# daisy9542/yolo-puncture

Hardware: AMD Instinct MI355X
Metric: images/sec (higher is better)
Workload: dtype bf16

## Files before the change

### include/yolop.h

```cpp
#ifndef YOLOP_H
#define YOLOP_H

#include <stddef.h>
#include <stdint.h>

#ifdef __cplusplus
extern "C" {
#endif

#define YP_OK 0
#define YP_ERR_ARG -1
#define YP_ERR_STATE -2
#define YP_ERR_HIP -3
#define YP_ERR_WEIGHT -4

#define YP_BF16 0
#define YP_F32 1

#define YP_TASK_DETECT 0
#define YP_TASK_SEGMENT 1

#define YP_NM 32
#define YP_MAX_MASKS 480
#define YP_MAX_DET 512
// ... 120 lines not shown
int yp_profile(yp_engine* e, const uint8_t* in_dev, int B, int H, int W, float* det_out, int32_t* idx_out,
               float* coeff_out, float* ms_out, int iters, void* stream);

int yp_set_nms(yp_engine* e, float conf, float iou);

int yp_set_attention_form(yp_engine* e, int form);

int yp_set_autotune(yp_engine* e, int enable);

int yp_tuning_export(const yp_engine* e, int32_t* cfg_out, int cap);
int yp_tuning_import(yp_engine* e, int B, int H, int W, const int32_t* cfg, int n);

int yp_debug_force_conv_cfg(int cfg);
int yp_debug_op_cfg(const yp_engine* e, int i, int* cfg);
int yp_debug_last_store_form(void);
int yp_debug_max_workgroups(int n);
int yp_debug_conv_families(int* base, int* num_cfgs, int cap);
int yp_debug_ablation(int v);
int yp_debug_head_clocks(uint64_t* out8);
int yp_debug_attention(const void* qkv_dev, void* o_dev, int dtype, int B, int N, int nh, int kd, int hd, int q_stride, int q_coff, int o_stride,
                       int o_coff, int wgs, int* kernel_out, void* stream);
int yp_debug_attention_form(const void* qkv_dev, void* o_dev, int dtype, int B, int N, int nh, int kd, int hd, int q_stride, int q_coff, int o_stride,
                            int o_coff, int wgs, int form, int* kernel_out, void* stream);
int yp_debug_topk_anchors(const uint32_t* const mk_dev[3], int B, const int hw[3][2], int k, int32_t* sel_out_dev, uint32_t* thr_out_dev, void* stream);
int yp_debug_head_branch_clocks(uint64_t* out8);
int yp_debug_head_winners(yp_engine* e, int32_t* sel_host, float* box_host, float* coeff_host);
int yp_debug_contour_clocks(uint64_t* out12);
int yp_debug_pwsp_clocks(uint64_t* out32);

int yp_tuning_source(const yp_engine* e);

int yp_debug_host_selftest(yp_engine* e);
int yp_debug_graph_info(const yp_engine* e, int64_t* out6);
int yp_debug_head_positions(yp_engine* e, int64_t* out6);
int yp_debug_marker(void* stream);

int yp_set_graph(yp_engine* e, int enable);

#ifdef __cplusplus
}
#endif
#endif
```

### yolo-puncture_amd/csrc/common.h

```cpp
#pragma once
#include <hip/hip_runtime.h>
#include <stdint.h>
#include <atomic>
#include <cstdlib>
#include <string>
#include <vector>

namespace yp {

enum DType { DT_BF16 = 0, DT_F32 = 1 };
enum Act { ACT_NONE = 0, ACT_SILU = 1, ACT_RELU = 2 };

enum OpKind {
    OP_STEM = 0,
    OP_CONV = 1,
    OP_DWCONV = 2,
    OP_POOL5 = 3,
    OP_UPSAMPLE = 4,
    OP_ATTN = 5,
    OP_HEAD = 6,
    OP_CONVT = 7,
    OP_AMAX = 9,
    OP_POOL3 = 8,
};
// ... 251 lines not shown
int conv_dma_requested_cfg(const ConvParams& p);
int conv_launch_cfg(const ConvParams& p, int dtype);
void conv_dma_force_cfg(int cfg);
int conv_dma_forced_cfg();
void conv_set_debug_ablation(int v);
int conv_debug_ablation();
bool tile_balance_enabled(int family);

struct ConvFamily {
    int base, num_cfgs;
    bool (*valid)(const ConvParams& p, int c);
    std::string (*symbol)(const ConvParams& p, int c);
    hipError_t (*launch)(const ConvParams& p, int c, hipStream_t st);
    bool two_source;
    const char* tune_env;
    bool opt_in;
};
inline const char* res_f32_args(const ConvParams& p) { return p.out_f32 ? ",false,true" : p.res ? ",true,false" : ",false,false"; }
extern const ConvFamily conv_dma_family, conv_halo_family, conv_halo_p_family, conv_dma_p_family, conv_dma_lc_family, conv_halo_s2_family,
    conv_tile1_family, conv_wreg_family, conv_pxd_family, conv_ks_family, conv_wres_family, conv_wrs_family;
constexpr int kNumConvFamilies = 12;
extern const ConvFamily* const kConvFamilies[kNumConvFamilies];
int conv_halo_s2_pw_cfg(const ConvParams& p);
hipError_t launch_dwconv(const DwParams& p, int dtype, hipStream_t st);
std::string dwconv_kernel_name(const DwParams& p, int dtype);
hipError_t launch_stem(const StemParams& p, int dtype, hipStream_t st);
std::string stem_kernel_name(const StemParams& p, int dtype);
hipError_t launch_pool5(const PoolParams& p, int dtype, hipStream_t st);
hipError_t launch_sppf_pool3(const PoolParams& p, int dtype, hipStream_t st);
bool sppf_pool3_fits(const PoolParams& p, int dtype);
bool dwconv_mfma_valid(const DwParams& p, int dtype);
hipError_t launch_dwconv_mfma(const DwParams& p, hipStream_t st);
const char* dwconv_mfma_kernel_name(const DwParams& p);
hipError_t launch_upsample(const UpParams& p, int dtype, hipStream_t st);
enum AttnForm { ATTN_FORM_AUTO = 0, ATTN_FORM_STREAM = 1, ATTN_FORM_STREAM_WIDE = 3 };
inline bool attn_form_valid(int form) { return form == ATTN_FORM_AUTO || form == ATTN_FORM_STREAM || form == ATTN_FORM_STREAM_WIDE; }
constexpr int ATTN_RESIDENT_TOKENS = 400;
hipError_t launch_attention(const AttnParams& p, int dtype, hipStream_t st, int wgs = 0, int* kernel_out = nullptr, int form = ATTN_FORM_AUTO);
bool attention_fits(const AttnParams& p, int dtype, int* max_tokens, int form = ATTN_FORM_AUTO);
bool attention_takes_stream(const AttnParams& p, int dtype, int form);
bool attention_takes_stream_wide(const AttnParams& p, int dtype, int form);
bool attention_stream_scope(const AttnParams& p, int dtype);
void attention_stream_split(int B, int N, int nh, int wgs, int* nsplit_out, int* gpw_out);
hipError_t launch_attention_stream(const AttnParams& p, hipStream_t st, int wgs);
bool attention_stream_wide_scope(const AttnParams& p, int dtype);
hipError_t launch_attention_stream_wide(const AttnParams& p, hipStream_t st, int wgs);
// ... 118 lines not shown
```

### yolo-puncture_amd/csrc/conv_halo_s2.hip

```cpp
#include "common.h"

namespace yp {

template <int FM, int FN, int WGM, int WGN, int NSH, bool HAS_RES, bool OUT_F32, bool PW2>
__global__ __launch_bounds__(WGM * WGN * 64) void conv_halo_s2_kernel(const ConvParams p, const int tiles_h, const int tiles_w,
                                                                    const int ntiles, const int G) {
    constexpr int NW = WGM * WGN;
    constexpr int TH = WGM * FM, BN = WGN * FN * 16;
    constexpr int HR = 2 * TH + 1;
    constexpr int HP = HR * 33;
    constexpr int H_INSTR = (HP * 4 + 63) / 64;
    constexpr int LH = (H_INSTR + NW - 1) / NW;
    constexpr int HB = H_INSTR * 1024;
    constexpr int S = FM * FN;
    static_assert(NSH == 3, "wait selection below is written for a 3-slot ring");
    static_assert((NSH - 2) * LH + 2 * S < 64, "vmcnt immediate");

    extern __shared__ __attribute__((aligned(1024))) unsigned char smem[];
    unsigned char* const Hs = smem;
    unsigned char* const dump = smem + NSH * HB;
    unsigned char* const Wres = dump + 1024;

    const int tid = threadIdx.x, lane = tid & 63;
    const int wave = __builtin_amdgcn_readfirstlane(tid >> 6);
    const int wm = wave % WGM, wn = wave / WGM;
    const int fr = lane & 15, fc = lane >> 4;
    const int nchunk = p.Cin >> 5;

    const int bid = xcd_remap(blockIdx.x, gridDim.x);
    const int nt = bid % ntiles, j0 = bid / ntiles;
    const int n0 = nt * BN;
    const int B = p.M / (p.Ho * p.Wo);
    const int num_tiles = B * tiles_h * tiles_w;

    const __amdgpu_buffer_rsrc_t xrs = __builtin_amdgcn_make_buffer_rsrc((void*)p.x, 0, (int)p.x_bytes, 0x00020000);
    const __amdgpu_buffer_rsrc_t wrs = __builtin_amdgcn_make_buffer_rsrc((void*)p.w, 0, (int)p.w_bytes, 0x00020000);
    const __amdgpu_buffer_rsrc_t yrs = __builtin_amdgcn_make_buffer_rsrc((void*)p.y, 0, (int)p.y_bytes, 0x00020000);

    float bias[FN][4];
#pragma unroll
    for (int a = 0; a < FN; ++a) {
        const int co = n0 + wn * (FN * 16) + a * 16 + fc * 4;
#pragma unroll
        for (int r = 0; r < 4; ++r) bias[a][r] = (co + r < p.Cout) ? p.bias[co + r] : 0.f;
    }

    {
        const int rows = 9 * nchunk * BN;
        const int ninstr = rows >> 4;
        for (int ii = wave; ii < ninstr; ii += NW) {
            const int s = ii * 64 + lane;
            const int rg = s >> 2, pc = s & 3;
            const int c8 = pc ^ cswz64(rg);
            const int n = rg % BN, q = rg / BN;
            const int tap = q % 9, ch = q / 9;
            const unsigned voff = (unsigned)(((n0 + n) * p.Kpad + tap * p.Cin + ch * 32 + c8 * 8) * 2);
            __builtin_amdgcn_raw_ptr_buffer_load_lds(wrs, (lds_void*)(Wres + ii * 1024), 16, voff, 0, 0, 0);
        }
    }

    unsigned char* const W2s = Wres + (size_t)9 * nchunk * BN * 64;
    float bias2[FN][4];
    if (PW2) {
        static_assert(!PW2 || BN == 64, "the fused trailing 1x1 is written for a 64-wide intermediate and output");
        const __amdgpu_buffer_rsrc_t w2rs = __builtin_amdgcn_make_buffer_rsrc((void*)p.w2, 0, (int)p.w2_bytes, 0x00020000);
        for (int ii = wave; ii < BN * 8 / 64; ii += NW) {
            const int s = ii * 64 + lane;
            const int row = s >> 3, pc = s & 7;
            const int c8 = pc ^ ((row >> 1) & 7);
            const unsigned voff = (unsigned)((row * p.Kpad2 + c8 * 8) * 2);
            __builtin_amdgcn_raw_ptr_buffer_load_lds(w2rs, (lds_void*)(W2s + ii * 1024), 16, voff, 0, 0, 0);
        }
#pragma unroll
        for (int a = 0; a < FN; ++a) {
            const int co = wn * (FN * 16) + a * 16 + fc * 4;
#pragma unroll
            for (int r = 0; r < 4; ++r) bias2[a][r] = (co + r < p.C2) ? p.bias2[co + r] : 0.f;
        }
    }

    unsigned hconst[LH];
// ... 30 lines not shown
        it_slot = (it_slot + 1 == NSH) ? 0 : it_slot + 1;
        if (++it_c == nchunk) {
            it_c = 0;
            it_tile += G;
            set_tile(it_tile);
        }
    };

#pragma unroll
    for (int s = 0; s < NSH - 1; ++s) issue_next();
    wait_vmcnt<0>();
    __builtin_amdgcn_s_barrier();

    int rd_slot = 0;
    unsigned epmask = 0;
    bool first_iter = true;
    for (int tile = j0; tile < num_tiles; tile += G) {
        f32x4 acc[FN][FM];
#pragma unroll
        for (int a = 0; a < FN; ++a)
#pragma unroll
            for (int r = 0; r < FM; ++r) acc[a][r] = f32x4{bias[a][0], bias[a][1], bias[a][2], bias[a][3]};

        for (int c = 0; c < nchunk; ++c) {
            if (!first_iter) {
                const int k = __builtin_popcount(epmask & ((1u << (NSH - 1)) - 1u));
                if (k == 0) wait_vmcnt<(NSH - 2) * LH>();
                else if (k == 1) wait_vmcnt<(NSH - 2) * LH + S>();
                else wait_vmcnt<(NSH - 2) * LH + 2 * S>();
                __builtin_amdgcn_s_barrier();
            }
            first_iter = false;
            issue_next();
            epmask <<= 1;

            const unsigned char* hsl = Hs + rd_slot * HB;
#pragma unroll
            for (int kx = 0; kx < 3; ++kx) {
                bf16x8 wf[3][FN];
#pragma unroll
                for (int ky = 0; ky < 3; ++ky)
#pragma unroll
                    for (int a = 0; a < FN; ++a) {
                        const int rw = (c * 9 + ky * 3 + kx) * BN + wn * (FN * 16) + a * 16 + fr;
                        wf[ky][a] = *(const bf16x8*)(Wres + swz64((unsigned)(rw * 64 + fc * 16)));
                    }
                const int eoff = (kx == 1) ? 17 + fr : fr + (kx >> 1);
#pragma unroll
                for (int jj = 0; jj < 2 * FM + 1; ++jj) {
                    const int hp = (2 * wm * FM + jj) * 33 + eoff;
                    const bf16x8 xf = *(const bf16x8*)(hsl + swz64((unsigned)(hp * 64 + fc * 16)));
                    if (jj & 1) {
#pragma unroll
                        for (int a = 0; a < FN; ++a)
                            acc[a][jj >> 1] = __builtin_amdgcn_mfma_f32_16x16x32_bf16(wf[1][a], xf, acc[a][jj >> 1], 0, 0, 0);
                    } else {
                        if ((jj >> 1) < FM) {
#pragma unroll
                            for (int a = 0; a < FN; ++a)
                                acc[a][jj >> 1] = __builtin_amdgcn_mfma_f32_16x16x32_bf16(wf[0][a], xf, acc[a][jj >> 1], 0, 0, 0);
                        }
                        if ((jj >> 1) >= 1) {
#pragma unroll
                            for (int a = 0; a < FN; ++a)
                                acc[a][(jj >> 1) - 1] = __builtin_amdgcn_mfma_f32_16x16x32_bf16(wf[2][a], xf, acc[a][(jj >> 1) - 1], 0, 0, 0);
                        }
                    }
                }
            }
            rd_slot = (rd_slot + 1 == NSH) ? 0 : rd_slot + 1;
        }

        if (PW2) {
            unsigned char* tb = Hs + ((rd_slot == 0) ? NSH - 1 : rd_slot - 1) * HB;
            __builtin_amdgcn_s_barrier();
#pragma unroll
            for (int r = 0; r < FM; ++r) {
                const int px = (wm * FM + r) * 16 + fr;
#pragma unroll
                for (int a = 0; a < FN; ++a) {
                    const int co = wn * (FN * 16) + a * 16 + fc * 4;
                    __attribute__((aligned(8))) __bf16 o[4];
                    float sv[4] = {acc[a][r][0], acc[a][r][1], acc[a][r][2], acc[a][r][3]};
                    if (p.act == ACT_SILU) silu4_packed(sv);
#pragma unroll
                    for (int i = 0; i < 4; ++i) o[i] = (__bf16)sv[i];
                    asm volatile("ds_write_b64 %0, %1" ::"v"((unsigned)(size_t)(__attribute__((address_space(3))) unsigned char*)(tb + px * 128 + (((co >> 3) ^ ((px >> 1) & 7)) * 16) + (co & 7) * 2)),
                                 "v"(*(const unsigned long long*)o) : "memory");
                }
            }
            asm volatile("s_waitcnt lgkmcnt(0)" ::: "memory");
            __builtin_amdgcn_s_barrier();
#pragma unroll
// ... 51 lines not shown
                    const int co = n0 + wn * (FN * 16) + a * 16 + fc * 4;
                    const bool ok = pix_ok && (co < (PW2 ? p.C2 : p.Cout));
                    float v[4] = {acc[a][r][0], acc[a][r][1], acc[a][r][2], acc[a][r][3]};
                    if ((PW2 ? p.act2 : p.act) == ACT_SILU) silu4_packed(v);
                    if (HAS_RES) {
                        const uint2 rr = rres[r][a];
                        add_res_bf16x4(v, rr);
                    }
                    if (OUT_F32) {
                        const unsigned off = ok ? (m * (unsigned)p.y_stride + (unsigned)(p.y_coff + co)) * 4u : kBufferOOB;
                        store_f32x4(v, yrs, off);
                    } else {
                        const unsigned off = ok ? (m * (unsigned)p.y_stride + (unsigned)(p.y_coff + co)) * 2u : kBufferOOB;
                        store_bf16x4(v, yrs, off);
                    }
                }
            }
        }
        epmask |= 1u;
    }
    wait_vmcnt<0>();
}

struct HaloS2Cfg { int FM, FN, WGM, WGN; const char* name; };
static const HaloS2Cfg kS2[] = {
    {2, 2, 4, 2, "conv_halo_s2_kernel<2,2,4,2,3"},
    {1, 2, 4, 2, "conv_halo_s2_kernel<1,2,4,2,3"},
    {2, 2, 4, 1, "conv_halo_s2_kernel<2,2,4,1,3"},
    {1, 2, 4, 1, "conv_halo_s2_kernel<1,2,4,1,3"},
    {2, 4, 4, 2, "conv_halo_s2_kernel<2,4,4,2,3"},
};
constexpr int kNumS2 = (int)(sizeof(kS2) / sizeof(kS2[0]));
static std::string conv_halo_s2_symbol(const ConvParams& p, int c) {
    return std::string(kS2[c].name) + (p.C2 > 0 ? ",false,false,true>" : std::string(res_f32_args(p)) + ",false>");
}

static size_t halo_s2_lds(const HaloS2Cfg& k, int Cin, bool pw2 = false) {
    const int TH = k.WGM * k.FM, BN = k.WGN * k.FN * 16;
    const int HP = (2 * TH + 1) * 33, H_INSTR = (HP * 4 + 63) / 64;
    return (size_t)3 * H_INSTR * 1024 + 1024 + (size_t)9 * (Cin / 32) * BN * 64 + (pw2 ? (size_t)BN * 128 : 0);
}

static bool conv_halo_s2_cfg_valid(const ConvParams& p, int c) {
    if (c < 0 || c >= kNumS2) return false;
    if (p.ks != 3 || p.stride != 2 || p.pad != 1 || p.up != 1 || (p.Cin % 32) != 0 || (p.Kpad != 9 * p.Cin)) return false;
    if ((p.H & 1) || (p.W & 1) || p.Ho * 2 != p.H || p.Wo * 2 != p.W) return false;
    if (p.x_bytes >= (1ull << 31) || p.w_bytes >= (1ull << 31) || p.y_bytes >= (1ull << 31)) return false;
    if ((p.Cout & 3) || (p.y_stride & 3) || (p.y_coff & 3) || (p.res && ((p.res_stride & 3) || (p.res_coff & 3)))) return false;
    if (p.res && p.out_f32) return false;
    const HaloS2Cfg& k = kS2[c];
    const int BN = k.WGN * k.FN * 16, TH = k.WGM * k.FM;
    const int cpad = (p.Cout + 31) / 32 * 32;
    if (BN > cpad) return false;
    if (halo_s2_lds(k, p.Cin) > 160 * 1024) return false;
    const long covered = (long)((p.Ho + TH - 1) / TH * TH) * ((p.Wo + 15) / 16 * 16);
    if (covered * 2 > (long)p.Ho * p.Wo * 3) return false;
    return true;
}

template <int FM, int FN, int WGM, int WGN, bool HAS_RES, bool OUT_F32, bool PW2 = false>
static hipError_t launch_halo_s2_var(const ConvParams& p, const HaloS2Cfg& k, hipStream_t st) {
    constexpr int TH = WGM * FM, BN = WGN * FN * 16;
    const size_t sh = halo_s2_lds(k, p.Cin, PW2);
    const int B = p.M / (p.Ho * p.Wo);
    const int tiles_h = (p.Ho + TH - 1) / TH, tiles_w = (p.Wo + 15) / 16, ntiles = (p.Cout + BN - 1) / BN;
    const int num_tiles = B * tiles_h * tiles_w;
    const int per_cu = (int)std::max<size_t>(1, std::min<size_t>(2, (160 * 1024) / sh));
    int G = (256 * per_cu) / ntiles;
    if (G < 1) G = 1;
    if (G > num_tiles) G = num_tiles;
    auto kern = conv_halo_s2_kernel<FM, FN, WGM, WGN, 3, HAS_RES, OUT_F32, PW2>;
    static size_t granted = 0;
    if (hipError_t e = allow_dynamic_lds((const void*)kern, sh, granted)) return e;
    hipLaunchKernelGGL(kern, dim3(G * ntiles), dim3(WGM * WGN * 64), sh, st, p, tiles_h, tiles_w, ntiles, G);
    return hipGetLastError();
}

template <int FM, int FN, int WGM, int WGN>
static hipError_t launch_halo_s2_one(const ConvParams& p, const HaloS2Cfg& k, hipStream_t st) {
    if (p.out_f32) return launch_halo_s2_var<FM, FN, WGM, WGN, false, true>(p, k, st);
    if (p.res) return launch_halo_s2_var<FM, FN, WGM, WGN, true, false>(p, k, st);
    return launch_halo_s2_var<FM, FN, WGM, WGN, false, false>(p, k, st);
}

int conv_halo_s2_pw_cfg(const ConvParams& p) {
    if (p.w2 == nullptr && p.C2 == 0) return -1;
    if (p.Cout != 64 || p.C2 != 64 || p.Kpad2 != 64 || p.res || p.out_f32) return -1;
    for (int c : {0, 1}) {
        ConvParams q = p;
        q.Cout = p.C2;
        if (!conv_halo_s2_cfg_valid(q, c)) continue;
        if (halo_s2_lds(kS2[c], p.Cin, true) > 160 * 1024) continue;
        return c;
    }
    return -1;
}

static hipError_t launch_conv_halo_s2(const ConvParams& p, int c, hipStream_t st) {
    const HaloS2Cfg& k = kS2[c];
    if (p.C2 > 0) {
        if (c == 0) return launch_halo_s2_var<2, 2, 4, 2, false, false, true>(p, k, st);
        if (c == 1) return launch_halo_s2_var<1, 2, 4, 2, false, false, true>(p, k, st);
        return hipErrorInvalidValue;
    }
    switch (c) {
        case 0: return launch_halo_s2_one<2, 2, 4, 2>(p, k, st);
        case 1: return launch_halo_s2_one<1, 2, 4, 2>(p, k, st);
        case 2: return launch_halo_s2_one<2, 2, 4, 1>(p, k, st);
        case 3: return launch_halo_s2_one<1, 2, 4, 1>(p, k, st);
        default: return launch_halo_s2_one<2, 4, 4, 2>(p, k, st);
    }
}

#if !defined(__HIP_DEVICE_COMPILE__)
const ConvFamily conv_halo_s2_family = {500, kNumS2, conv_halo_s2_cfg_valid, conv_halo_s2_symbol, launch_conv_halo_s2, false, "YOLOP_NO_S2", false};
#endif

}
```

### yolo-puncture_amd/csrc/engine.hip

```cpp
#include "../../include/yolop.h"
#include "common.h"
#include <algorithm>
#include <array>
#include <chrono>

#include <cmath>
#include <cstdarg>
#include <cstdio>
#include <cstring>
#include <cstdlib>
#include <dlfcn.h>
#include <fcntl.h>
#include <fstream>
#include <map>
#include <sstream>
#include <memory>

using namespace yp;

static thread_local char g_err[512] = "";
static int fail(int code, const char* fmt, ...) {
    va_list ap;
    va_start(ap, fmt);
    vsnprintf(g_err, sizeof(g_err), fmt, ap);
// ... 2348 lines not shown
        return fail(YP_ERR_ARG, "yp_debug_attention: the output slice [%d, %lld) does not fit o_stride = %d", o_coff, (long long)o_coff + (long long)nh * hd, o_stride);
    if ((q_stride | q_coff | o_stride | o_coff) & 3)
        return fail(YP_ERR_ARG, "yp_debug_attention: strides and channel offsets must be multiples of 4 elements (q_stride %d, q_coff %d, o_stride %d, o_coff %d)",
                    q_stride, q_coff, o_stride, o_coff);
    AttnParams p{};
    p.qkv = qkv_dev; p.q_stride = q_stride; p.q_coff = q_coff; p.o = o_dev; p.o_stride = o_stride; p.o_coff = o_coff;
    p.B = B; p.N = N; p.nh = nh; p.kd = kd; p.hd = hd; p.scale = 1.0f / std::sqrt((float)kd);
    int max_tokens = 0;
    if (!attention_fits(p, dtype, &max_tokens, form))
        return fail(YP_ERR_ARG, "yp_debug_attention: no kernel for N = %d, kd = %d, hd = %d: the attention kernels hold at most %d tokens and want kd and hd in multiples of 4",
                    N, kd, hd, max_tokens);
    hipStream_t st = (hipStream_t)stream;
    hipError_t err = launch_attention(p, dtype, st, wgs, kernel_out, form);
    if (err == hipSuccess) err = hipStreamSynchronize(st);
    if (err != hipSuccess) return fail(YP_ERR_HIP, "yp_debug_attention: %s", hipGetErrorString(err));
    return YP_OK;
}

int yp_debug_attention(const void* qkv_dev, void* o_dev, int dtype, int B, int N, int nh, int kd, int hd, int q_stride, int q_coff, int o_stride,
                       int o_coff, int wgs, int* kernel_out, void* stream) {
    return yp_debug_attention_form(qkv_dev, o_dev, dtype, B, N, nh, kd, hd, q_stride, q_coff, o_stride, o_coff, wgs, ATTN_FORM_AUTO, kernel_out, stream);
}

int yp_tuning_source(const yp_engine* e) {
    if (!e) return YP_ERR_ARG;
    return e->tune_source;
}

int yp_debug_graph_info(const yp_engine* e, int64_t* out6) {
    if (!e || !out6) return fail(YP_ERR_ARG, "yp_debug_graph_info: null argument");
    out6[0] = e->n_captures; out6[1] = e->g_nodes; out6[2] = e->g_edges; out6[3] = e->g_edges_expected;
    out6[4] = (int64_t)e->lanes_used.size() + 1; out6[5] = e->gexec ? 1 : 0;
    return YP_OK;
}

int yp_debug_head_positions(yp_engine* e, int64_t* out6) {
    if (!e || !out6) return fail(YP_ERR_ARG, "yp_debug_head_positions: null argument");
    for (int i = 0; i < 6; ++i) out6[i] = 0;
    if (!e->allocated) return fail(YP_ERR_STATE, "no forward has run yet");
    const Op* h = nullptr;
    for (const Op& o : e->ops) if (o.kind == OP_HEAD) h = &o;
    if (!h || !(h->sparse_box || h->sparse_cf) || !e->sp_ws) return 0;
    HIPCHK(hipSetDevice(e->device));
    HIPCHK(hipDeviceSynchronize());
    const SparseWs ws = sparse_ws_layout(*e);
    const char* base = (const char*)e->sp_ws;
// ... 366 lines not shown
```

### yolo-puncture_amd/engine.py

```python
from __future__ import annotations

import ctypes as C
import os
from typing import Dict, List, Optional, Tuple

import numpy as np
import torch

from .weights import fold_state

_LIB: Optional[C.CDLL] = None
_HERE = os.path.dirname(os.path.abspath(__file__))
LIB_PATH = os.environ.get("YOLOP_LIB") or os.path.join(_HERE, "libyolop.so")

YP_BF16, YP_F32 = 0, 1
TASK_DETECT, TASK_SEGMENT = 0, 1
OP_KINDS = {0: "stem", 1: "conv", 2: "dwconv", 3: "pool5", 4: "upsample", 5: "attn", 6: "head", 7: "convT", 8: "pool3", 9: "amax"}
FORMS = ("plain", "dwpw", "dwpw_tail", "s2pw", "frontend", "c2f", "scdown", "pwsp", "cls_out")


class ModelDesc(C.Structure):
    _fields_ = [("variant", C.c_int), ("nc", C.c_int), ("task", C.c_int), ("dtype", C.c_int), ("max_det", C.c_int), ("family", C.c_int)]


# ... 21 lines not shown
    lib.yp_forward.argtypes = [vp, vp, C.c_int, C.c_int, C.c_int, vp, vp, vp, vp]
    lib.yp_proto.argtypes = [vp, C.POINTER(vp), ip, ip]
    lib.yp_masks.argtypes = [vp, C.c_int, vp, vp, C.c_int, C.c_int, C.c_int, C.c_int, vp, vp, vp, C.c_int, C.c_int, vp]
    lib.yp_id_mask_resized.argtypes = [vp, C.c_int, vp, vp] + [C.c_int] * 5 + [vp, vp, C.c_int, C.c_int, vp]
    lib.yp_id_mask_resized.restype = C.c_int
    lib.yp_mask_contours.argtypes = [vp, C.c_int, C.c_int, C.c_int, C.c_int, vp, vp, vp, vp]
    lib.yp_mask_contours.restype = C.c_int
    lib.yp_mask_contours_scaled.argtypes = [vp, C.c_int, C.c_int, C.c_int, C.c_int, C.c_int, vp, vp, vp, C.c_int, vp, C.c_int, C.c_int, vp]
    lib.yp_mask_contours_scaled.restype = C.c_int
    lib.yp_mask_contours_large_workspace.argtypes = [C.c_int, C.c_int, C.c_int]
    lib.yp_mask_contours_large_workspace.restype = C.c_size_t
    lib.yp_mask_contours_large.argtypes = [vp, C.c_int, C.c_int, C.c_int, C.c_int, C.c_int, vp, vp, vp, C.c_int, vp, C.c_int, C.c_int, C.c_int, vp,
                                           C.c_size_t, vp]
    lib.yp_mask_contours_large.restype = C.c_int
    lib.yp_plan.argtypes = [vp, C.c_int, C.c_int, C.c_int]
    lib.yp_max_batch.argtypes = [vp, C.c_int, C.c_int]
    lib.yp_max_batch.restype = C.c_int
    lib.yp_debug_topk_anchors.argtypes = [C.POINTER(vp), C.c_int, C.POINTER(C.c_int), C.c_int, vp, vp, vp]
    lib.yp_debug_topk_anchors.restype = C.c_int
    lib.yp_debug_attention.argtypes = [vp, vp] + [C.c_int] * 11 + [ip, vp]
    lib.yp_debug_attention.restype = C.c_int
    lib.yp_debug_attention_form.argtypes = [vp, vp] + [C.c_int] * 12 + [ip, vp]
    lib.yp_debug_attention_form.restype = C.c_int
    lib.yp_set_attention_form.argtypes = [vp, C.c_int]
    lib.yp_set_attention_form.restype = C.c_int
    lib.yp_op_info.argtypes = [vp, C.c_int, C.c_char_p, C.c_int, ip, C.POINTER(C.c_double), C.POINTER(C.c_double)]
    lib.yp_op_output.argtypes = [vp, C.c_int, ip, ip, ip]
    lib.yp_op_kernel.argtypes = [vp, C.c_int, C.c_char_p, C.c_int]
    lib.yp_op_fusion.argtypes = [vp, C.c_int, ip, ip]
    lib.yp_op_fusion.restype = C.c_int
    lib.yp_debug_op_form.argtypes = [vp, C.c_int, ip, ip, C.c_int]
    lib.yp_debug_op_form.restype = C.c_int
    lib.yp_run_op.argtypes = [vp, C.c_int, vp, vp, vp, vp, vp]
    lib.yp_tensor_write.argtypes = [vp, C.c_int, C.c_int, C.c_int, vp]
    lib.yp_tensor_count.argtypes = [vp]
    lib.yp_tensor_info.argtypes = [vp, C.c_int, C.c_char_p, C.c_int, ip, ip]
    lib.yp_tensor_read.argtypes = [vp, C.c_int, vp]
    lib.yp_profile.argtypes = [vp, vp, C.c_int, C.c_int, C.c_int, vp, vp, vp, vp, C.c_int, vp]
    lib.yp_set_graph.argtypes = [vp, C.c_int]
    lib.yp_set_autotune.argtypes = [vp, C.c_int]
    lib.yp_set_nms.argtypes = [vp, C.c_float, C.c_float]
    lib.yp_set_nms.restype = C.c_int
    lib.yp_debug_host_selftest.argtypes = [vp]
    lib.yp_debug_host_selftest.restype = C.c_int
    lib.yp_tuning_source.argtypes = [vp]
    lib.yp_tuning_source.restype = C.c_int
# ... 24 lines not shown
    lib.yp_masks_frames.argtypes = [vp, vp, C.c_int, vp, C.c_long, vp, C.c_int, C.c_int, vp, vp]
    lib.yp_masks_frames.restype = C.c_int
    lib.yp_masks_frames_input.argtypes = [vp, vp, C.c_int, vp, C.c_long, vp, C.c_int, C.c_int, vp, vp]
    lib.yp_masks_frames_input.restype = C.c_int
    lib.yp_comm_unique_id.argtypes = [vp]
    lib.yp_comm_create.argtypes = [vp, C.c_int, C.c_int, C.c_int, C.POINTER(vp)]
    lib.yp_allgather.argtypes = [vp, vp, vp, C.c_size_t, vp]
    lib.yp_comm_destroy.argtypes = [vp]
    for fn in ("yp_comm_unique_id", "yp_comm_create", "yp_allgather", "yp_comm_destroy"):
        getattr(lib, fn).restype = C.c_int
    for fn in ("yp_create", "yp_destroy", "yp_weight_count", "yp_weight_info", "yp_set_weight", "yp_finalize",
               "yp_forward", "yp_proto", "yp_masks", "yp_plan", "yp_op_info", "yp_op_output", "yp_op_input", "yp_tensor_count",
               "yp_tensor_info", "yp_tensor_read", "yp_profile", "yp_set_graph", "yp_run_op", "yp_tensor_write",
               "yp_op_kernel", "yp_set_autotune", "yp_debug_force_conv_cfg", "yp_debug_ablation"):
        getattr(lib, fn).restype = C.c_int
    if path is None:
        _LIB = lib
    return lib


EXPORTS = ["yp_last_error", "yp_create", "yp_destroy", "yp_weight_count", "yp_weight_info", "yp_set_weight",
           "yp_finalize", "yp_forward", "yp_proto", "yp_masks", "yp_id_mask_resized", "yp_plan", "yp_op_info", "yp_op_output", "yp_op_input", "yp_op_fusion",
           "yp_tensor_count", "yp_tensor_info", "yp_tensor_read", "yp_profile", "yp_set_graph", "yp_run_op",
           "yp_tensor_write", "yp_op_kernel", "yp_set_autotune", "yp_tuning_export", "yp_tuning_import", "yp_set_nms", "yp_debug_force_conv_cfg", "yp_debug_op_cfg", "yp_debug_op_form", "yp_debug_last_store_form", "yp_debug_max_workgroups", "yp_debug_conv_families", "yp_debug_ablation", "yp_debug_head_clocks", "yp_debug_head_branch_clocks", "yp_debug_head_winners", "yp_debug_contour_clocks", "yp_debug_pwsp_clocks", "yp_debug_host_selftest", "yp_debug_graph_info", "yp_tuning_source", "yp_debug_head_positions", "yp_debug_marker", "yp_max_batch", "yp_debug_topk_anchors", "yp_debug_attention", "yp_debug_attention_form", "yp_set_attention_form", "yp_letterbox", "yp_letterbox_batch", "yp_masks_frames", "yp_masks_frames_input", "yp_mask_contours",
           "yp_mask_contours_scaled", "yp_mask_contours_large_workspace", "yp_mask_contours_large", "yp_comm_unique_id", "yp_comm_create", "yp_allgather", "yp_comm_destroy",
           "yp_u2net_create", "yp_u2net_destroy", "yp_u2net_weight_count", "yp_u2net_weight_info", "yp_u2net_set_weight", "yp_u2net_finalize",
           "yp_u2net_forward", "yp_u2net_forward_crops", "yp_u2net_set_graph", "yp_u2net_tensor_count", "yp_u2net_tensor_info", "yp_u2net_tensor_read",
           "yp_u2net_op_count", "yp_u2net_op_info",
           "yp_cls_create", "yp_cls_destroy", "yp_cls_weight_count", "yp_cls_weight_info", "yp_cls_set_weight", "yp_cls_finalize",
           "yp_cls_forward", "yp_cls_set_graph", "yp_cls_tensor_count", "yp_cls_tensor_info", "yp_cls_tensor_read"]


MAX_ANCHORS = 294912
ATTENTION_FORMS = {"auto": 0, "stream": 1, "stream_wide": 3}


def _attention_form(form) -> int:
    if form not in ATTENTION_FORMS:
        raise ValueError(f"attention form {form!r}: one of {sorted(ATTENTION_FORMS)}")
    return ATTENTION_FORMS[form]


def topk_anchors(mk: List[torch.Tensor], hw, k: int) -> Tuple[torch.Tensor, torch.Tensor]:
    lib = load_library()
    if len(mk) != 3 or len(hw) != 3:
        raise ValueError("three levels")
    B = int(mk[0].shape[0])
# ... 8 lines not shown
    rc = lib.yp_debug_topk_anchors(ptrs, B, hwa, int(k), C.c_void_p(sel.data_ptr()), C.c_void_p(thr.data_ptr()), C.c_void_p(_stream_ptr(dev)))
    if rc < 0:
        raise YolopError(lib.yp_last_error().decode())
    return sel, thr


def attention(qkv: torch.Tensor, nh: int, kd: int, hd: int, q_coff: int = 0, out: Optional[torch.Tensor] = None, o_coff: int = 0,
              wgs: int = 0, form: str = "auto") -> Tuple[torch.Tensor, int]:
    lib = load_library()
    if qkv.dim() != 3 or qkv.dtype not in (torch.bfloat16, torch.float32) or not qkv.is_contiguous() or not qkv.is_cuda:
        raise ValueError("qkv must be a contiguous device bf16 / float32 [B, N, q_stride]")
    B, N, q_stride = (int(v) for v in qkv.shape)
    if out is None:
        out = torch.empty((B, N, int(nh) * int(hd)), dtype=qkv.dtype, device=qkv.device)
    if out.dim() != 3 or out.dtype != qkv.dtype or not out.is_contiguous() or out.device != qkv.device or tuple(out.shape[:2]) != (B, N):
        raise ValueError("out must be a contiguous [B, N, o_stride] of qkv's dtype on its device")
    kernel = C.c_int(-1)
    rc = lib.yp_debug_attention_form(C.c_void_p(qkv.data_ptr()), C.c_void_p(out.data_ptr()), YP_BF16 if qkv.dtype == torch.bfloat16 else YP_F32, B, N,
                                int(nh), int(kd), int(hd), q_stride, int(q_coff), int(out.shape[2]), int(o_coff), int(wgs), _attention_form(form), C.byref(kernel),
                                C.c_void_p(_stream_ptr(qkv.device)))
    if rc < 0:
        raise YolopError(lib.yp_last_error().decode())
    return out, kernel.value


def conv_families() -> List[Tuple[int, int]]:
    lib = load_library()
    n = lib.yp_debug_conv_families(None, None, 0)
    base, num = (C.c_int * n)(), (C.c_int * n)()
    lib.yp_debug_conv_families(base, num, n)
    return list(zip(base, num))


def _stream_ptr(device: torch.device) -> int:
    return int(torch.cuda.current_stream(device).cuda_stream)


def letterbox_device(src: torch.Tensor, geo: dict, out: Optional[torch.Tensor] = None, pad_value: int = 114) -> torch.Tensor:
    if not (src.is_cuda and src.dtype == torch.uint8 and src.dim() == 3 and src.shape[2] == 3 and src.is_contiguous()):
        raise ValueError("letterbox_device needs a contiguous uint8 CUDA tensor [H,W,3]")
    oh, ow = int(geo["out_h"]), int(geo["out_w"])
    if out is None:
        out = torch.empty((oh, ow, 3), dtype=torch.uint8, device=src.device)
    if not (out.is_cuda and out.dtype == torch.uint8 and tuple(out.shape) == (oh, ow, 3) and out.is_contiguous()):
        raise ValueError(f"letterbox_device: output must be a contiguous uint8 CUDA tensor [{oh},{ow},3]")
    lib = load_library()
# ... 403 lines not shown
```

Measured before the change: 23330.

## Hold stride-2 halo conv weights in registers for small Cin

Adds register-resident weight variants of the stride-2 halo conv for Cin of 32 or 64. These variants stage weights through LDS once and keep them in VGPRs, then unroll the chunk loop. The dynamic LDS footprint shrinks to roughly the halo ring, and per-tap LDS weight reads in the inner loop go away. The variants are selected by default for cfg 0/1 when no fused pointwise is present. The trade is up to 144 extra VGPRs, which can lower occupancy, and per_cu is forced to 1 when sizing the grid.

```diff
diff --git a/include/yolop.h b/include/yolop.h
--- a/include/yolop.h
+++ b/include/yolop.h
@@ -166,6 +166,9 @@
                        int o_coff, int wgs, int* kernel_out, void* stream);
 int yp_debug_attention_form(const void* qkv_dev, void* o_dev, int dtype, int B, int N, int nh, int kd, int hd, int q_stride, int q_coff, int o_stride,
                             int o_coff, int wgs, int form, int* kernel_out, void* stream);
+int yp_debug_conv_s2(const void* x_dev, const void* w_dev, const float* bias_dev, const void* res_dev, void* y_dev, int out_f32, int B, int H,
+                     int W, int Cin, int Cout, int silu, int cfg, int lds_weights, int64_t* lds_out, char* kernel_out, int kernel_cap,
+                     void* stream);
 int yp_debug_topk_anchors(const uint32_t* const mk_dev[3], int B, const int hw[3][2], int k, int32_t* sel_out_dev, uint32_t* thr_out_dev, void* stream);
 int yp_debug_head_branch_clocks(uint64_t* out8);
 int yp_debug_head_winners(yp_engine* e, int32_t* sel_host, float* box_host, float* coeff_host);
diff --git a/yolo-puncture_amd/csrc/common.h b/yolo-puncture_amd/csrc/common.h
--- a/yolo-puncture_amd/csrc/common.h
+++ b/yolo-puncture_amd/csrc/common.h
@@ -297,6 +297,8 @@
 constexpr int kNumConvFamilies = 12;
 extern const ConvFamily* const kConvFamilies[kNumConvFamilies];
 int conv_halo_s2_pw_cfg(const ConvParams& p);
+size_t conv_halo_s2_lds_bytes(const ConvParams& p, int c);
+int conv_halo_s2_lds_weights(int on);
 hipError_t launch_dwconv(const DwParams& p, int dtype, hipStream_t st);
 std::string dwconv_kernel_name(const DwParams& p, int dtype);
 hipError_t launch_stem(const StemParams& p, int dtype, hipStream_t st);
diff --git a/yolo-puncture_amd/csrc/conv_halo_s2.hip b/yolo-puncture_amd/csrc/conv_halo_s2.hip
--- a/yolo-puncture_amd/csrc/conv_halo_s2.hip
+++ b/yolo-puncture_amd/csrc/conv_halo_s2.hip
@@ -2,9 +2,10 @@
 
 namespace yp {
 
-template <int FM, int FN, int WGM, int WGN, int NSH, bool HAS_RES, bool OUT_F32, bool PW2>
-__global__ __launch_bounds__(WGM * WGN * 64) void conv_halo_s2_kernel(const ConvParams p, const int tiles_h, const int tiles_w,
-                                                                    const int ntiles, const int G) {
+constexpr int kS2WregMaxVgprs = 144;
+
+template <int FM, int FN, int WGM, int WGN, int NSH, bool HAS_RES, bool OUT_F32, bool PW2, int NCH>
+__device__ __forceinline__ void conv_halo_s2_body(const ConvParams& p, const int tiles_h, const int tiles_w, const int ntiles, const int G) {
     constexpr int NW = WGM * WGN;
     constexpr int TH = WGM * FM, BN = WGN * FN * 16;
     constexpr int HR = 2 * TH + 1;
@@ -13,6 +14,8 @@
     constexpr int LH = (H_INSTR + NW - 1) / NW;
     constexpr int HB = H_INSTR * 1024;
     constexpr int S = FM * FN;
+    constexpr bool WREG = NCH > 0;
+    static_assert(!WREG || (!PW2 && 9 * NCH * FN * 4 <= kS2WregMaxVgprs), "register-weights form");
     static_assert(NSH == 3, "wait selection below is written for a 3-slot ring");
     static_assert((NSH - 2) * LH + 2 * S < 64, "vmcnt immediate");
 
@@ -25,7 +28,7 @@
     const int wave = __builtin_amdgcn_readfirstlane(tid >> 6);
     const int wm = wave % WGM, wn = wave / WGM;
     const int fr = lane & 15, fc = lane >> 4;
-    const int nchunk = p.Cin >> 5;
+    const int nchunk = WREG ? NCH : p.Cin >> 5;
 
     const int bid = xcd_remap(blockIdx.x, gridDim.x);
     const int nt = bid % ntiles, j0 = bid / ntiles;
@@ -45,7 +48,7 @@
         for (int r = 0; r < 4; ++r) bias[a][r] = (co + r < p.Cout) ? p.bias[co + r] : 0.f;
     }
 
-    {
+    if constexpr (!WREG) {
         const int rows = 9 * nchunk * BN;
         const int ninstr = rows >> 4;
         for (int ii = wave; ii < ninstr; ii += NW) {
@@ -57,6 +60,38 @@
             const unsigned voff = (unsigned)(((n0 + n) * p.Kpad + tap * p.Cin + ch * 32 + c8 * 8) * 2);
             __builtin_amdgcn_raw_ptr_buffer_load_lds(wrs, (lds_void*)(Wres + ii * 1024), 16, voff, 0, 0, 0);
         }
+    }
+    bf16x8 wr[WREG ? NCH : 1][9][FN];
+    if constexpr (WREG) {
+        constexpr int W_INSTR = 9 * BN / 16;
+#pragma unroll
+        for (int c = 0; c < NCH; ++c) {
+            for (int ii = wave; ii < W_INSTR; ii += NW) {
+                const int s = ii * 64 + lane;
+                const int rg = s >> 2, pc = s & 3;
+                const int c8 = pc ^ cswz64(rg);
+                const int tap = rg / BN, n = rg - tap * BN;
+                const unsigned voff = (unsigned)(((n0 + n) * p.Kpad + tap * p.Cin + c * 32 + c8 * 8) * 2);
+                __builtin_amdgcn_raw_ptr_buffer_load_lds(wrs, (lds_void*)(Hs + ii * 1024), 16, voff, 0, 0, 0);
+            }
+            wait_vmcnt<0>();
+            __builtin_amdgcn_s_barrier();
+#pragma unroll
+            for (int t = 0; t < 9; ++t)
+#pragma unroll
+                for (int a = 0; a < FN; ++a) {
+                    const int rw = t * BN + wn * (FN * 16) + a * 16 + fr;
+                    wr[c][t][a] = *(const bf16x8*)(Hs + swz64((unsigned)(rw * 64 + fc * 16)));
+                }
+            __builtin_amdgcn_s_waitcnt(0xc07f);
+            __builtin_amdgcn_s_barrier();
+        }
+#pragma unroll
+        for (int c = 0; c < NCH; ++c)
+#pragma unroll
+            for (int t = 0; t < 9; ++t)
+#pragma unroll
+                for (int a = 0; a < FN; ++a) asm volatile("" : "+v"(wr[c][t][a]));
     }
 
     unsigned char* const W2s = Wres + (size_t)9 * nchunk * BN * 64;
@@ -133,7 +168,7 @@
 #pragma unroll
             for (int r = 0; r < FM; ++r) acc[a][r] = f32x4{bias[a][0], bias[a][1], bias[a][2], bias[a][3]};
 
-        for (int c = 0; c < nchunk; ++c) {
+        auto chunk = [&](const int c) {
             if (!first_iter) {
                 const int k = __builtin_popcount(epmask & ((1u << (NSH - 1)) - 1u));
                 if (k == 0) wait_vmcnt<(NSH - 2) * LH>();
@@ -153,8 +188,12 @@
                 for (int ky = 0; ky < 3; ++ky)
 #pragma unroll
                     for (int a = 0; a < FN; ++a) {
-                        const int rw = (c * 9 + ky * 3 + kx) * BN + wn * (FN * 16) + a * 16 + fr;
-                        wf[ky][a] = *(const bf16x8*)(Wres + swz64((unsigned)(rw * 64 + fc * 16)));
+                        if constexpr (WREG) {
+                            wf[ky][a] = wr[c][ky * 3 + kx][a];
+                        } else {
+                            const int rw = (c * 9 + ky * 3 + kx) * BN + wn * (FN * 16) + a * 16 + fr;
+                            wf[ky][a] = *(const bf16x8*)(Wres + swz64((unsigned)(rw * 64 + fc * 16)));
+                        }
                     }
                 const int eoff = (kx == 1) ? 17 + fr : fr + (kx >> 1);
 #pragma unroll
@@ -180,6 +219,12 @@
                 }
             }
             rd_slot = (rd_slot + 1 == NSH) ? 0 : rd_slot + 1;
+        };
+        if constexpr (WREG) {
+#pragma unroll
+            for (int c = 0; c < NCH; ++c) chunk(c);
+        } else {
+            for (int c = 0; c < nchunk; ++c) chunk(c);
         }
 
         if (PW2) {
@@ -277,23 +322,56 @@
     wait_vmcnt<0>();
 }
 
-struct HaloS2Cfg { int FM, FN, WGM, WGN; const char* name; };
+template <int FM, int FN, int WGM, int WGN, int NSH, bool HAS_RES, bool OUT_F32, bool PW2>
+__global__ __launch_bounds__(WGM * WGN * 64) void conv_halo_s2_kernel(const ConvParams p, const int tiles_h, const int tiles_w,
+                                                                    const int ntiles, const int G) {
+    conv_halo_s2_body<FM, FN, WGM, WGN, NSH, HAS_RES, OUT_F32, PW2, 0>(p, tiles_h, tiles_w, ntiles, G);
+}
+template <int FM, int FN, int WGM, int WGN, int NSH, bool HAS_RES, bool OUT_F32, bool PW2, int NCH>
+__global__ __launch_bounds__(WGM * WGN * 64) void conv_halo_s2_kernel(const ConvParams p, const int tiles_h, const int tiles_w,
+                                                                    const int ntiles, const int G) {
+    static_assert(NCH > 0, "the ninth argument is a register-weights form's chunk count");
+    conv_halo_s2_body<FM, FN, WGM, WGN, NSH, HAS_RES, OUT_F32, PW2, NCH>(p, tiles_h, tiles_w, ntiles, G);
+}
+
+struct HaloS2Cfg { int FM, FN, WGM, WGN; const char* name; bool wreg; };
 static const HaloS2Cfg kS2[] = {
-    {2, 2, 4, 2, "conv_halo_s2_kernel<2,2,4,2,3"},
-    {1, 2, 4, 2, "conv_halo_s2_kernel<1,2,4,2,3"},
-    {2, 2, 4, 1, "conv_halo_s2_kernel<2,2,4,1,3"},
-    {1, 2, 4, 1, "conv_halo_s2_kernel<1,2,4,1,3"},
-    {2, 4, 4, 2, "conv_halo_s2_kernel<2,4,4,2,3"},
+    {2, 2, 4, 2, "conv_halo_s2_kernel<2,2,4,2,3", false},
+    {1, 2, 4, 2, "conv_halo_s2_kernel<1,2,4,2,3", false},
+    {2, 2, 4, 1, "conv_halo_s2_kernel<2,2,4,1,3", false},
+    {1, 2, 4, 1, "conv_halo_s2_kernel<1,2,4,1,3", false},
+    {2, 4, 4, 2, "conv_halo_s2_kernel<2,4,4,2,3", false},
+    {1, 2, 4, 2, "conv_halo_s2_kernel<1,2,4,2,3", true},
+    {2, 2, 4, 2, "conv_halo_s2_kernel<2,2,4,2,3", true},
+    {2, 2, 2, 4, "conv_halo_s2_kernel<2,2,2,4,3", true},
 };
-constexpr int kNumS2 = (int)(sizeof(kS2) / sizeof(kS2[0]));
+constexpr int kNumS2 = 5;
+constexpr int kNumS2Forms = (int)(sizeof(kS2) / sizeof(kS2[0]));
+
+static std::atomic<int>& s2_lds_weights_ref() {
+    static std::atomic<int> v{env_on("YOLOP_S2_LDS_WEIGHTS") ? 1 : 0};
+    return v;
+}
+int conv_halo_s2_lds_weights(int on) { return on < 0 ? s2_lds_weights_ref().load() : s2_lds_weights_ref().exchange(on ? 1 : 0); }
+
+static int halo_s2_form(const ConvParams& p, int c) {
+    if (c > 1 || p.C2 > 0 || s2_lds_weights_ref().load()) return c;
+    if ((p.Cin % 32) != 0 || 9 * (p.Cin / 32) * 2 * 4 > kS2WregMaxVgprs) return c;
+    if (c == 0) return 6;
+    return p.Cout > 96 ? 7 : 5;
+}
 static std::string conv_halo_s2_symbol(const ConvParams& p, int c) {
-    return std::string(kS2[c].name) + (p.C2 > 0 ? ",false,false,true>" : std::string(res_f32_args(p)) + ",false>");
+    const HaloS2Cfg& k = kS2[halo_s2_form(p, c)];
+    if (k.wreg) return std::string(k.name) + res_f32_args(p) + ",false," + std::to_string(p.Cin / 32) + ">";
+    return std::string(k.name) + (p.C2 > 0 ? ",false,false,true>" : std::string(res_f32_args(p)) + ",false>");
 }
 
 static size_t halo_s2_lds(const HaloS2Cfg& k, int Cin, bool pw2 = false) {
     const int TH = k.WGM * k.FM, BN = k.WGN * k.FN * 16;
     const int HP = (2 * TH + 1) * 33, H_INSTR = (HP * 4 + 63) / 64;
-    return (size_t)3 * H_INSTR * 1024 + 1024 + (size_t)9 * (Cin / 32) * BN * 64 + (pw2 ? (size_t)BN * 128 : 0);
+    const size_t ring = (size_t)3 * H_INSTR * 1024 + 1024;
+    if (k.wreg) return std::max(ring, (size_t)9 * BN * 64);
+    return ring + (size_t)9 * (Cin / 32) * BN * 64 + (pw2 ? (size_t)BN * 128 : 0);
 }
 
 static bool conv_halo_s2_cfg_valid(const ConvParams& p, int c) {
@@ -303,7 +381,7 @@
     if (p.x_bytes >= (1ull << 31) || p.w_bytes >= (1ull << 31) || p.y_bytes >= (1ull << 31)) return false;
     if ((p.Cout & 3) || (p.y_stride & 3) || (p.y_coff & 3) || (p.res && ((p.res_stride & 3) || (p.res_coff & 3)))) return false;
     if (p.res && p.out_f32) return false;
-    const HaloS2Cfg& k = kS2[c];
+    const HaloS2Cfg& k = kS2[halo_s2_form(p, c)];
     const int BN = k.WGN * k.FN * 16, TH = k.WGM * k.FM;
     const int cpad = (p.Cout + 31) / 32 * 32;
     if (BN > cpad) return false;
@@ -313,22 +391,36 @@
     return true;
 }
 
-template <int FM, int FN, int WGM, int WGN, bool HAS_RES, bool OUT_F32, bool PW2 = false>
+template <int FM, int FN, int WGM, int WGN, bool HAS_RES, bool OUT_F32, bool PW2 = false, int... WCH>
 static hipError_t launch_halo_s2_var(const ConvParams& p, const HaloS2Cfg& k, hipStream_t st) {
     constexpr int TH = WGM * FM, BN = WGN * FN * 16;
     const size_t sh = halo_s2_lds(k, p.Cin, PW2);
     const int B = p.M / (p.Ho * p.Wo);
     const int tiles_h = (p.Ho + TH - 1) / TH, tiles_w = (p.Wo + 15) / 16, ntiles = (p.Cout + BN - 1) / BN;
     const int num_tiles = B * tiles_h * tiles_w;
-    const int per_cu = (int)std::max<size_t>(1, std::min<size_t>(2, (160 * 1024) / sh));
+    const int per_cu = sizeof...(WCH) > 0 ? 1 : (int)std::max<size_t>(1, std::min<size_t>(2, (160 * 1024) / sh));
     int G = (256 * per_cu) / ntiles;
     if (G < 1) G = 1;
     if (G > num_tiles) G = num_tiles;
-    auto kern = conv_halo_s2_kernel<FM, FN, WGM, WGN, 3, HAS_RES, OUT_F32, PW2>;
+    auto kern = conv_halo_s2_kernel<FM, FN, WGM, WGN, 3, HAS_RES, OUT_F32, PW2, WCH...>;
     static size_t granted = 0;
     if (hipError_t e = allow_dynamic_lds((const void*)kern, sh, granted)) return e;
     hipLaunchKernelGGL(kern, dim3(G * ntiles), dim3(WGM * WGN * 64), sh, st, p, tiles_h, tiles_w, ntiles, G);
     return hipGetLastError();
+}
+
+template <int FM, int FN, int WGM, int WGN, int NCH>
+static hipError_t launch_halo_s2_wreg_n(const ConvParams& p, const HaloS2Cfg& k, hipStream_t st) {
+    if (p.out_f32) return launch_halo_s2_var<FM, FN, WGM, WGN, false, true, false, NCH>(p, k, st);
+    if (p.res) return launch_halo_s2_var<FM, FN, WGM, WGN, true, false, false, NCH>(p, k, st);
+    return launch_halo_s2_var<FM, FN, WGM, WGN, false, false, false, NCH>(p, k, st);
+}
+template <int FM, int FN, int WGM, int WGN>
+static hipError_t launch_halo_s2_wreg(const ConvParams& p, const HaloS2Cfg& k, hipStream_t st) {
+    static_assert(FN == 2 && 9 * 2 * FN * 4 <= kS2WregMaxVgprs && 9 * 3 * FN * 4 > kS2WregMaxVgprs, "the chunk counts instantiated below are those halo_s2_form admits");
+    if (p.Cin == 32) return launch_halo_s2_wreg_n<FM, FN, WGM, WGN, 1>(p, k, st);
+    if (p.Cin == 64) return launch_halo_s2_wreg_n<FM, FN, WGM, WGN, 2>(p, k, st);
+    return hipErrorInvalidValue;
 }
 
 template <int FM, int FN, int WGM, int WGN>
@@ -351,19 +443,28 @@
     return -1;
 }
 
+size_t conv_halo_s2_lds_bytes(const ConvParams& p, int c) { return (c >= 0 && c < kNumS2) ? halo_s2_lds(kS2[halo_s2_form(p, c)], p.Cin) : 0; }
+
 static hipError_t launch_conv_halo_s2(const ConvParams& p, int c, hipStream_t st) {
-    const HaloS2Cfg& k = kS2[c];
+    if (c < 0 || c >= kNumS2) return hipErrorInvalidValue;
+    const int form = halo_s2_form(p, c);
+    const HaloS2Cfg& k = kS2[form];
     if (p.C2 > 0) {
         if (c == 0) return launch_halo_s2_var<2, 2, 4, 2, false, false, true>(p, k, st);
         if (c == 1) return launch_halo_s2_var<1, 2, 4, 2, false, false, true>(p, k, st);
         return hipErrorInvalidValue;
     }
-    switch (c) {
+    static_assert(kNumS2Forms == 8, "one case per entry of kS2");
+    switch (form) {
         case 0: return launch_halo_s2_one<2, 2, 4, 2>(p, k, st);
         case 1: return launch_halo_s2_one<1, 2, 4, 2>(p, k, st);
         case 2: return launch_halo_s2_one<2, 2, 4, 1>(p, k, st);
         case 3: return launch_halo_s2_one<1, 2, 4, 1>(p, k, st);
-        default: return launch_halo_s2_one<2, 4, 4, 2>(p, k, st);
+        case 4: return launch_halo_s2_one<2, 4, 4, 2>(p, k, st);
+        case 5: return launch_halo_s2_wreg<1, 2, 4, 2>(p, k, st);
+        case 6: return launch_halo_s2_wreg<2, 2, 4, 2>(p, k, st);
+        case 7: return launch_halo_s2_wreg<2, 2, 2, 4>(p, k, st);
+        default: return hipErrorInvalidValue;
     }
 }
 
diff --git a/yolo-puncture_amd/csrc/engine.hip b/yolo-puncture_amd/csrc/engine.hip
--- a/yolo-puncture_amd/csrc/engine.hip
+++ b/yolo-puncture_amd/csrc/engine.hip
@@ -2394,6 +2394,47 @@
     return yp_debug_attention_form(qkv_dev, o_dev, dtype, B, N, nh, kd, hd, q_stride, q_coff, o_stride, o_coff, wgs, ATTN_FORM_AUTO, kernel_out, stream);
 }
 
+int yp_debug_conv_s2(const void* x_dev, const void* w_dev, const float* bias_dev, const void* res_dev, void* y_dev, int out_f32, int B, int H,
+                     int W, int Cin, int Cout, int silu, int cfg, int lds_weights, int64_t* lds_out, char* kernel_out, int kernel_cap, void* stream) {
+    if (lds_out) *lds_out = 0;
+    if (kernel_out && kernel_cap > 0) kernel_out[0] = 0;
+    const bool host_only = !x_dev && !w_dev && !bias_dev && !y_dev;
+    if (!host_only && (!x_dev || !w_dev || !bias_dev || !y_dev)) return fail(YP_ERR_ARG, "yp_debug_conv_s2: null argument");
+    if (B < 1 || H < 2 || W < 2 || Cin < 1 || Cout < 1)
+        return fail(YP_ERR_ARG, "yp_debug_conv_s2: non-positive size (B %d, H %d, W %d, Cin %d, Cout %d)", B, H, W, Cin, Cout);
+    const ConvFamily& f = conv_halo_s2_family;
+    if (cfg < f.base || cfg >= f.base + f.num_cfgs)
+        return fail(YP_ERR_ARG, "yp_debug_conv_s2: cfg = %d is no id of the stride-2 halo family [%d, %d)", cfg, f.base, f.base + f.num_cfgs);
+    const size_t esz = out_f32 ? 4 : 2;
+    ConvParams p{};
+    p.x = x_dev; p.x_stride = Cin; p.x_coff = 0; p.H = H; p.W = W; p.Cin = Cin;
+    p.w = w_dev; p.Kpad = 9 * Cin; p.bias = bias_dev;
+    p.Ho = H / 2; p.Wo = W / 2; p.Cout = Cout;
+    p.y = y_dev; p.y_stride = Cout; p.y_coff = 0;
+    p.res = res_dev; p.res_stride = Cout; p.res_coff = 0;
+    p.M = B * p.Ho * p.Wo;
+    p.ks = 3; p.stride = 2; p.pad = 1; p.up = 1;
+    p.act = silu ? ACT_SILU : ACT_NONE; p.out_f32 = out_f32 ? 1 : 0;
+    p.x_bytes = (size_t)B * H * W * Cin * 2; p.w_bytes = (size_t)Cout * 9 * Cin * 2; p.y_bytes = (size_t)p.M * Cout * esz;
+    p.cfg = -1;
+    const int before = conv_halo_s2_lds_weights(lds_weights ? 1 : 0);
+    const bool ok = f.valid(p, cfg - f.base);
+    hipError_t err = hipSuccess;
+    if (lds_out) *lds_out = (int64_t)conv_halo_s2_lds_bytes(p, cfg - f.base);
+    if (ok && kernel_out && kernel_cap > 0) std::snprintf(kernel_out, (size_t)kernel_cap, "%s", f.symbol(p, cfg - f.base).c_str());
+    if (ok && !host_only) {
+        hipStream_t st = (hipStream_t)stream;
+        err = f.launch(p, cfg - f.base, st);
+        if (err == hipSuccess) err = hipStreamSynchronize(st);
+    }
+    conv_halo_s2_lds_weights(before);
+    if (!ok)
+        return fail(YP_ERR_ARG, "yp_debug_conv_s2: configuration %d does not admit B %d, H %d, W %d, Cin %d, Cout %d%s%s%s", cfg, B, H, W, Cin, Cout,
+                    res_dev ? ", residual" : "", out_f32 ? ", fp32 output" : "", lds_weights ? ", weights in LDS" : "");
+    if (err != hipSuccess) return fail(YP_ERR_HIP, "yp_debug_conv_s2: %s", hipGetErrorString(err));
+    return YP_OK;
+}
+
 int yp_tuning_source(const yp_engine* e) {
     if (!e) return YP_ERR_ARG;
     return e->tune_source;
diff --git a/yolo-puncture_amd/engine.py b/yolo-puncture_amd/engine.py
--- a/yolo-puncture_amd/engine.py
+++ b/yolo-puncture_amd/engine.py
@@ -67,6 +67,8 @@
     lib.yp_debug_attention.restype = C.c_int
     lib.yp_debug_attention_form.argtypes = [vp, vp] + [C.c_int] * 12 + [ip, vp]
     lib.yp_debug_attention_form.restype = C.c_int
+    lib.yp_debug_conv_s2.argtypes = [vp, vp, vp, vp, vp] + [C.c_int] * 9 + [C.POINTER(C.c_int64), C.c_char_p, C.c_int, vp]
+    lib.yp_debug_conv_s2.restype = C.c_int
     lib.yp_set_attention_form.argtypes = [vp, C.c_int]
     lib.yp_set_attention_form.restype = C.c_int
     lib.yp_op_info.argtypes = [vp, C.c_int, C.c_char_p, C.c_int, ip, C.POINTER(C.c_double), C.POINTER(C.c_double)]
@@ -137,7 +139,7 @@
 EXPORTS = ["yp_last_error", "yp_create", "yp_destroy", "yp_weight_count", "yp_weight_info", "yp_set_weight",
            "yp_finalize", "yp_forward", "yp_proto", "yp_masks", "yp_id_mask_resized", "yp_plan", "yp_op_info", "yp_op_output", "yp_op_input", "yp_op_fusion",
            "yp_tensor_count", "yp_tensor_info", "yp_tensor_read", "yp_profile", "yp_set_graph", "yp_run_op",
-           "yp_tensor_write", "yp_op_kernel", "yp_set_autotune", "yp_tuning_export", "yp_tuning_import", "yp_set_nms", "yp_debug_force_conv_cfg", "yp_debug_op_cfg", "yp_debug_op_form", "yp_debug_last_store_form", "yp_debug_max_workgroups", "yp_debug_conv_families", "yp_debug_ablation", "yp_debug_head_clocks", "yp_debug_head_branch_clocks", "yp_debug_head_winners", "yp_debug_contour_clocks", "yp_debug_pwsp_clocks", "yp_debug_host_selftest", "yp_debug_graph_info", "yp_tuning_source", "yp_debug_head_positions", "yp_debug_marker", "yp_max_batch", "yp_debug_topk_anchors", "yp_debug_attention", "yp_debug_attention_form", "yp_set_attention_form", "yp_letterbox", "yp_letterbox_batch", "yp_masks_frames", "yp_masks_frames_input", "yp_mask_contours",
+           "yp_tensor_write", "yp_op_kernel", "yp_set_autotune", "yp_tuning_export", "yp_tuning_import", "yp_set_nms", "yp_debug_force_conv_cfg", "yp_debug_op_cfg", "yp_debug_op_form", "yp_debug_last_store_form", "yp_debug_max_workgroups", "yp_debug_conv_families", "yp_debug_ablation", "yp_debug_head_clocks", "yp_debug_head_branch_clocks", "yp_debug_head_winners", "yp_debug_contour_clocks", "yp_debug_pwsp_clocks", "yp_debug_host_selftest", "yp_debug_graph_info", "yp_tuning_source", "yp_debug_head_positions", "yp_debug_marker", "yp_max_batch", "yp_debug_topk_anchors", "yp_debug_attention", "yp_debug_attention_form", "yp_debug_conv_s2", "yp_set_attention_form", "yp_letterbox", "yp_letterbox_batch", "yp_masks_frames", "yp_masks_frames_input", "yp_mask_contours",
            "yp_mask_contours_scaled", "yp_mask_contours_large_workspace", "yp_mask_contours_large", "yp_comm_unique_id", "yp_comm_create", "yp_allgather", "yp_comm_destroy",
            "yp_u2net_create", "yp_u2net_destroy", "yp_u2net_weight_count", "yp_u2net_weight_info", "yp_u2net_set_weight", "yp_u2net_finalize",
            "yp_u2net_forward", "yp_u2net_forward_crops", "yp_u2net_set_graph", "yp_u2net_tensor_count", "yp_u2net_tensor_info", "yp_u2net_tensor_read",
@@ -192,6 +194,38 @@
     if rc < 0:
         raise YolopError(lib.yp_last_error().decode())
     return out, kernel.value
+
+
+def conv_s2(x: torch.Tensor, w: torch.Tensor, bias: torch.Tensor, cfg: int, res: Optional[torch.Tensor] = None, out_f32: bool = False,
+            silu: bool = True, lds_weights: bool = False) -> torch.Tensor:
+    lib = load_library()
+    if x.dim() != 4 or w.dim() != 4 or x.dtype != torch.bfloat16 or w.dtype != torch.bfloat16 or bias.dtype != torch.float32:
+        raise ValueError("x: bf16 [B, H, W, Cin], w: bf16 [Cout, 3, 3, Cin], bias: float32 [Cout]")
+    B, H, W, Cin = (int(v) for v in x.shape)
+    Cout = int(w.shape[0])
+    if tuple(w.shape) != (Cout, 3, 3, Cin) or tuple(bias.shape) != (Cout,) or not (x.is_cuda and w.is_cuda and bias.is_cuda):
+        raise ValueError("w must be [Cout, 3, 3, Cin] and bias [Cout], all on the device")
+    if not (x.is_contiguous() and w.is_contiguous() and bias.is_contiguous()):
+        raise ValueError("contiguous tensors")
+    if res is not None and (res.dtype != torch.bfloat16 or tuple(res.shape) != (B, H // 2, W // 2, Cout) or not res.is_contiguous() or res.device != x.device):
+        raise ValueError("res must be a contiguous bf16 [B, H/2, W/2, Cout] on x's device")
+    y = torch.zeros((B, H // 2, W // 2, Cout), dtype=torch.float32 if out_f32 else torch.bfloat16, device=x.device)
+    rc = lib.yp_debug_conv_s2(C.c_void_p(x.data_ptr()), C.c_void_p(w.data_ptr()), C.c_void_p(bias.data_ptr()),
+                              C.c_void_p(res.data_ptr()) if res is not None else None, C.c_void_p(y.data_ptr()), int(bool(out_f32)), B, H, W, Cin, Cout,
+                              int(bool(silu)), int(cfg), int(bool(lds_weights)), None, None, 0, C.c_void_p(_stream_ptr(x.device)))
+    if rc < 0:
+        raise YolopError(lib.yp_last_error().decode())
+    return y
+
+
+def conv_s2_admits(cfg: int, B: int, H: int, W: int, Cin: int, Cout: int, res: bool = False, out_f32: bool = False,
+                   lds_weights: bool = False) -> Tuple[bool, int, str]:
+    lib = load_library()
+    lds = C.c_int64(0)
+    name = C.create_string_buffer(160)
+    rc = lib.yp_debug_conv_s2(None, None, None, C.c_void_p(1) if res else None, None, int(bool(out_f32)), int(B), int(H), int(W), int(Cin), int(Cout),
+                              1, int(cfg), int(bool(lds_weights)), C.byref(lds), name, 160, None)
+    return rc >= 0, int(lds.value), name.value.decode()
 
 
 def conv_families() -> List[Tuple[int, int]]:
```

Measured after the change: 23590, median of 6. +1.1%, better.
